# daxiongpro/EPNet

Hardware: AMD Instinct MI355X
Metric: SA-stack points/sec per GPU (16384-pt KITTI scene) + % HBM roofline (higher is better)
Workload: dtype f32; 1 GPU; 256 x 16384-pt kitti scenes per GPU per step through the 4-level SA op stack (4 samplings [FPS + centre gather; levels 2-4 nested in level 1 where tie-free] + 8 ball_query + 8 fused groupings [xyz - centre ; features]), pyramid 16384>4096>1024>256>64, radii [[.1,.5],[.5,1],[1,2],[2,4]], nsample [16,32], C=0/96/256/512, HIP-graph launch; levels=4, scenes_per_gpu=256, software_pipelined=True, pipeline_stages=2, parallelism=scene-parallel x1

## Files before the change

### epnet_amd/_lib.py

```python
import contextlib
import ctypes
import os

_HERE = os.path.dirname(os.path.abspath(__file__))
LIB_PATH = os.environ.get("EPNET_HIP_LIB") or os.path.join(_HERE, "lib", "libepnet_hip.so")

_vp = ctypes.c_void_p
_i = ctypes.c_int
_f = ctypes.c_float
_d = ctypes.c_double
_sz = ctypes.c_size_t
_i64 = ctypes.c_int64

SIGNATURES = {
    "epnet_abi_version": (_i, []),
    "epnet_strerror": (ctypes.c_char_p, [_i]),
    "epnet_last_hip_error": (ctypes.c_char_p, []),
    "epnet_set_tuning": (_i, [ctypes.c_char_p, _i]),
    "epnet_get_tuning": (_i, [ctypes.c_char_p, ctypes.POINTER(_i)]),
    "epnet_furthest_point_sampling": (_i, [_i, _i, _i, _vp, _vp, _vp, _vp]),
    "epnet_gather_points": (_i, [_i, _i, _i, _i, _vp, _vp, _vp, _vp]),
    "epnet_gather_points_grad": (_i, [_i, _i, _i, _i, _vp, _vp, _vp, _vp]),
    "epnet_ball_query": (_i, [_i, _i, _i, _f, _i, _vp, _vp, _vp, _vp]),
    "epnet_ball_query_workspace_bytes": (_sz, [_i, _i, _i]),
# ... 31 lines not shown
    "epnet_group_linear_grad_w_det_workspace_bytes": (_sz, [_i, _i, _i, _i]),
    "epnet_group_linear_grad_w_det": (_i, [_i, _i, _i, _i, _i, _vp, _vp, _vp, _vp, _vp, _vp, _sz, _vp]),
    "epnet_pool_max": (_i, [ctypes.c_longlong, _i, _vp, _vp, _vp, _vp]),
    "epnet_pool_max_grad": (_i, [ctypes.c_longlong, _i, _vp, _vp, _vp, _vp]),
    "epnet_group_linear_h": (_i, [_i, _i, _i, _i, _i, _vp, _vp, _vp, _vp, _vp, _vp, _vp, _i, _vp]),
    "epnet_pool_max_h": (_i, [ctypes.c_longlong, _i, _vp, _vp, _vp, _i, _vp]),
    "epnet_pool_max_grad_h": (_i, [ctypes.c_longlong, _i, _vp, _vp, _vp, _i, _vp]),
    "epnet_three_interpolate_h": (_i, [_i, _i, _i, _i, _vp, _vp, _vp, _vp, _i, _vp]),
    "epnet_scene_index_bytes": (_sz, [_i, _i]),
    "epnet_scene_index_build": (_i, [_i, _i, _vp, _vp, _sz, _vp]),
    "epnet_scene_index_build_gathered": (_i, [_i, _i, _i, _vp, _vp, _vp, _vp, _sz, _vp]),
    "epnet_furthest_point_sampling_indexed": (_i, [_i, _i, _i, _vp, _vp, _sz, _vp, _vp, _vp]),
    "epnet_sample_centres": (_i, [_i, _i, _i, _vp, _vp, _sz, _vp, _vp, _vp, _vp]),
    "epnet_sample_centres_chain": (_i, [_i, _i, _i, _vp, _vp, _sz, _vp, _vp, _vp, _vp, _vp, _i, _vp]),
    "epnet_sample_centres_chain_index": (_i, [_i, _i, _i, _vp, _vp, _sz, _vp, _vp, _vp, _vp, _vp, _i, _vp, _sz, _vp]),
    "epnet_group_concat_multi": (_i, [_i, _i, _i, _i, _i, _vp, _vp, _vp, _vp, _vp, _vp, _i, _vp]),
    "epnet_ball_query_indexed_multi": (_i, [_i, _i, _i, _i, _vp, _vp, _vp, _vp, _vp, _sz, _vp, _vp]),
    "epnet_ball_query_ordered": (_i, [_i, _i, _i, _i, _vp, _vp, _vp, _vp, _vp, _sz, _vp, _sz, _vp, _vp]),
    "epnet_three_nn_indexed": (_i, [_i, _i, _i, _vp, _vp, _vp, _sz, _vp, _sz, _vp, _vp, _vp]),
    "epnet_ball_query_indexed": (_i, [_i, _i, _i, _f, _i, _vp, _vp, _vp, _sz, _vp, _vp]),
    "epnet_boxes_overlap_bev": (_i, [_i, _vp, _i, _vp, _vp, _vp]),
    "epnet_boxes_iou_bev": (_i, [_i, _vp, _i, _vp, _vp, _vp]),
    "epnet_boxes_iou3d": (_i, [_i, _vp, _i, _vp, _vp, _vp]),
    "epnet_boxes_iou3d_pairs": (_i, [_i, _vp, _vp, _vp, _vp]),
    "epnet_aug_roi_by_noise": (_i, [_i, _i, _f, _vp, _vp, _vp, _vp, _vp, _vp, _vp, _vp]),
    "epnet_rcnn_sample_rois_workspace_bytes": (_sz, [_i, _i, _i, _i]),
    "epnet_rcnn_sample_rois": (_i, [_i, _i, _i, _i, _i, _i, _f, _f, _f, _d, _i, _vp, _vp, _vp, _vp, _vp, _vp, _vp, _sz, _vp, _vp, _vp,
                                    _vp, _vp, _vp, _vp, _vp, _vp, _vp]),
    "epnet_rpn_proposals_workspace_bytes": (_sz, [_i, _i, _i, _i]),
    "epnet_rpn_proposals": (_i, [_i, _i, _vp, _vp, _vp, _i, _i, _i, _f, _i, _vp, _sz, _vp, _vp, _vp, _vp]),
# ... 95 lines not shown
```

### epnet_amd/csrc/fps.hip

```cpp
#include <math.h>

#include <type_traits>

#include "common.h"
#include "dpp.h"
#include "spatial.h"

extern "C" __device__ int epnet_llvm_writelane_i32(int, int, int) __asm("llvm.amdgcn.writelane.i32");

namespace epnet {

__device__ __forceinline__ int writelane_i32(int value, int lane, int old) {
    return epnet_llvm_writelane_i32(value, lane, old);
}

__device__ __forceinline__ unsigned bitrev_lg(unsigned v, int lg) {
    return lg == 0 ? 0u : (__brev(v) >> (32 - lg));
}

__device__ __forceinline__ int wave_max_i32(int v) {
    const int r = row16_max(v);
    const int a = __builtin_amdgcn_readlane(r, 0), b = __builtin_amdgcn_readlane(r, 16);
    const int c = __builtin_amdgcn_readlane(r, 32), d = __builtin_amdgcn_readlane(r, 48);
    return max(max(a, b), max(c, d));
// ... 271 lines not shown
    if (PPT <= 8) a |= a >> 8;
    return (unsigned)a & (PPT >= 32 ? 0xFFFFFFFFu : ((1u << PPT) - 1u));
}

constexpr int kIdxBufP = 1024;

template <typename VH>
__device__ __forceinline__ unsigned rank_of(const VH &rk2, int j) {
    return ((unsigned)rk2[j >> 1] >> ((j & 1) << 4)) & 0xFFFFu;
}
template <typename VH>
__device__ __forceinline__ void set_rank(VH &rk2, int j, unsigned r) {
    rk2[j >> 1] = (j & 1) ? (int)(((unsigned)rk2[j >> 1] & 0xFFFFu) | (r << 16)) : (int)r;
}

template <int kW, int PPT, typename VF, typename VI, typename VH>
__device__ __forceinline__ void fps_rounds(unsigned long long *s_key, float4 (*s_rec)[64 * kW], int *s_idx, int m, const VF &x,
                                           const VF &y, const VF &z, VI &t, const VH &rk2,
                                           float cx, float cy, float cz, int *__restrict__ idxs,
                                           int *__restrict__ tie_free = nullptr, int known = 0,
                                           const float *__restrict__ xyz_in_order = nullptr, int detect_upto = 0x7fffffff) {
    const int q = threadIdx.x;
    const int lane = q & 63, wave = q >> 6;
    const int sub = lane & (PPT - 1);
    const int kNeg1 = __float_as_int(-1.f);

    int bm = kNeg1;
    float lox = 0.f, hix = 0.f, loy = 0.f, hiy = 0.f, loz = 0.f, hiz = 0.f;
    for (int j = 0; j < PPT; ++j) {
        const float xj = x[j], yj = y[j], zj = z[j];
        const int tj = t[j];
        const bool real = tj != kNeg1;
        const float mnx = group_minf<PPT>(real ? xj : 3.4e38f), mxx = group_maxf<PPT>(real ? xj : -3.4e38f);
        const float mny = group_minf<PPT>(real ? yj : 3.4e38f), mxy = group_maxf<PPT>(real ? yj : -3.4e38f);
        const float mnz = group_minf<PPT>(real ? zj : 3.4e38f), mxz = group_maxf<PPT>(real ? zj : -3.4e38f);
        const int gm = group_max<PPT>(tj);
        if (sub == j) {
            const bool any = gm != kNeg1;
            bm = gm;
            lox = any ? mnx : 0.f; hix = any ? mxx : 0.f;
            loy = any ? mny : 0.f; hiy = any ? mxy : 0.f;
            loz = any ? mnz : 0.f; hiz = any ? mxz : 0.f;
        }
    }
    if (q < 3) s_key[q] = 0ull;
    if (q == 0) s_idx[0] = 0;
    if (known > kIdxBufP || known > m || !xyz_in_order) known = 0;
    for (int i = q; i < known; i += 64 * kW) s_idx[i] = (int)rank14(i);
    __syncthreads();
    for (int it = 1; it < known; ++it) {
        const float px = __builtin_amdgcn_fmed3f(cx, lox, hix), py = __builtin_amdgcn_fmed3f(cy, loy, hiy),
                    pz = __builtin_amdgcn_fmed3f(cz, loz, hiz);
        const float bdx = px - cx, bdy = py - cy, bdz = pz - cz;
        const float L = bdx * bdx + bdy * bdy + bdz * bdz;
        unsigned active = fold_parts<PPT>(__ballot(__float_as_int(L) < bm));
        const float nx = xyz_in_order[it * 3 + 0], ny = xyz_in_order[it * 3 + 1], nz = xyz_in_order[it * 3 + 2];
        while (active) {
            const int j = (int)__builtin_ctz(active);
            active &= active - 1u;
            const float xj = x[j], yj = y[j], zj = z[j];
            const int told = t[j];
            __builtin_amdgcn_sched_barrier(0);
// ... 8 lines not shown
        cy = ny;
        cz = nz;
    }

    __builtin_amdgcn_s_setprio(EPNET_FPS_PRIO);
    EPNET_STATS_BEGIN;
    EPNET_STAMP(t_loop0);
    bool stale = true;
    int wbest = kNeg1;
    unsigned long long hbuckets = 0ull;
    unsigned racc = 0xFFFFFFFFu;
    float xa = 0.f, ya = 0.f, za = 0.f;
    int kb = 1;
    bool wave_multi = false;
    int tied_v = 0x7fffffff;
    auto round = [&](auto ties_tag, const int it) __attribute__((always_inline)) {
        constexpr bool kTies = decltype(ties_tag)::value;
        EPNET_STAMP(t0);
        const float px = __builtin_amdgcn_fmed3f(cx, lox, hix), py = __builtin_amdgcn_fmed3f(cy, loy, hiy),
                    pz = __builtin_amdgcn_fmed3f(cz, loz, hiz);
        const float bdx = px - cx, bdy = py - cy, bdz = pz - cz;
        const float L = bdx * bdx + bdy * bdy + bdz * bdz;
        const unsigned long long act64 = __ballot(__float_as_int(L) < bm);
        unsigned active = fold_parts<PPT>(act64);
        EPNET_CNT(0, __popc(active));
        stale = stale || __ballot((hbuckets & act64) != 0ull) != 0ull;
        EPNET_STAMP(t1);
        while (active) {
            const int j = (int)__builtin_ctz(active);
            active &= active - 1u;
            const float xj = x[j], yj = y[j], zj = z[j];
            const int told = t[j];
            __builtin_amdgcn_sched_barrier(0);
            const float dx = xj - cx, dy = yj - cy, dz = zj - cz;
            const float d = dx * dx + dy * dy + dz * dz;
            const int tj = min(__float_as_int(d), told);
            t[j] = tj;
            const int gm = group_max<PPT>(tj);
            bm = (sub == j) ? gm : bm;
        }
        EPNET_STAMP(t2);
        if (stale) {
            stale = false;
            wbest = wave_max_all(bm);
            unsigned cand = fold_parts<PPT>(__ballot(bm == wbest));
            racc = 0xFFFFFFFFu;
            hbuckets = 0ull;
            do {
                const int j = (int)__builtin_ctz(cand);
                cand &= cand - 1u;
                const int tj = t[j];
                const float xj = x[j], yj = y[j], zj = z[j];
                const unsigned rw = (unsigned)rk2[j >> 1];
                __builtin_amdgcn_sched_barrier(0);
                const unsigned r = tj == wbest ? ((rw >> ((j & 1) << 4)) & 0xFFFFu) : 0xFFFFFFFFu;
                if (r != 0xFFFFFFFFu) hbuckets |= 1ull << ((lane & ~(PPT - 1)) | j);
// ... 33 lines not shown
            const int wd = (int)(unsigned)(kfull >> 32);
            const bool suspect = (wbest == wd && (!mine || wave_multi)) || wd == 0;
            if (__builtin_amdgcn_readfirstlane(suspect ? 1 : 0)) {
                bool differs = false;
                const unsigned mine_slots = (unsigned)((hbuckets >> (lane & ~(PPT - 1))) & ((1ull << PPT) - 1ull));
                unsigned any_slots = mine_slots;
                for (int off = 32; off >= 1; off >>= 1) any_slots |= (unsigned)__shfl_xor((int)any_slots, off, 64);
#pragma unroll 1
                while (any_slots) {
                    const int j = (int)__builtin_ctz(any_slots);
                    any_slots &= any_slots - 1u;
                    const float xj = x[j], yj = y[j], zj = z[j];
                    __builtin_amdgcn_sched_barrier(0);
                    differs = differs || (((mine_slots >> j) & 1u) && (xj != cx || yj != cy || zj != cz));
                }
                if (wd == 0 || __ballot(differs)) tied_v = min(tied_v, it);
            }
        }
        const int kb2 = kb == 0 ? 2 : kb - 1;
        kb = kb == 2 ? 0 : kb + 1;
        if (wave == 0) {
            s_idx[it & (kIdxBufP - 1)] = (int)(0x3FFFu - (klo >> 10));
            if (lane == 0) s_key[kb2] = 0ull;
            if ((it & (kIdxBufP - 1)) == kIdxBufP - 1) {
                const int base = it - (kIdxBufP - 1);
                for (int e = lane; e < kIdxBufP; e += 64) idxs[base + e] = unrank14((unsigned)s_idx[e]);
            }
        }
        EPNET_STAMP(t5);
        EPNET_ACC(1, t0, t1); EPNET_ACC(2, t1, t2); EPNET_ACC(3, t2, t3); EPNET_ACC(4, t3, t4); EPNET_ACC(5, t4, t5);
    };
    int it0 = max(1, known);
    if (tie_free) {
        const int upto = min(m, detect_upto);
        for (; it0 < upto; ++it0) round(std::true_type{}, it0);
    }
    for (; it0 < m; ++it0) round(std::false_type{}, it0);
    EPNET_STAMP(t_loop1);
    EPNET_ACC(6, t_loop0, t_loop1);
    EPNET_STATS_END;
    if (tie_free && lane == 0) atomicMin(tie_free, min(min(tied_v, m), detect_upto));
    if (wave == 0) {
        const int base = (m - 1) & ~(kIdxBufP - 1);
        for (int e = lane; base + e < m; e += 64) idxs[base + e] = unrank14((unsigned)s_idx[e]);
    }
}

template <int kW, int PPT>
__global__ __launch_bounds__(64 * kW) void fps_pruned_kernel(int n, int m, const float *__restrict__ xyz,
                                                             float *__restrict__ temp, int *__restrict__ idxs,
                                                             const int *__restrict__ skip, int *__restrict__ prefix_out,
                                                             int prefix_cap) {
// ... 58 lines not shown

template <int kT, int BITS, int kPer, int kStage>
__device__ __attribute__((noinline)) void fps_index_epilogue(int *s_hist, float (*s_box)[16], int *s_part, int m, int np,
                                                             const float *xyz, float4 *sorted, float *boxes, float *qboxes, int n_src,
                                                             const int *src_idx, float *gathered) {
    scene_index_build_block<kT, BITS, kPer, kStage, true>(s_hist, s_box, s_part, m, np, xyz, sorted, boxes, qboxes, n_src, src_idx,
                                                          gathered);
}

template <int kW, int PPT>
__global__ __launch_bounds__(64 * kW) void fps_indexed_kernel(int n, int m, const float4 *__restrict__ sorted,
                                                              float *__restrict__ temp, int *__restrict__ idxs,
                                                              const int *__restrict__ prefix_in,
                                                              int *__restrict__ prefix_out, const float *__restrict__ xyz,
                                                              int prefix_cap, int prologue_init, void *next_index,
                                                              float *__restrict__ new_xyz) {
    typedef float vecf __attribute__((ext_vector_type(PPT)));
    typedef int veci __attribute__((ext_vector_type(PPT)));
    constexpr int NP = 64 * kW * PPT;
    constexpr bool kEpilogue = kW == 8;
    constexpr int kRecAt = 0, kIdxAt = kRecAt + 2 * 64 * kW * 16, kKeyAt = kIdxAt + kIdxBufP * 4, kFirstAt = kKeyAt + 32,
                  kRoundsBytes = kFirstAt + 16;
    constexpr int kIxBits = 12, kIxPer = 8, kIxStage = 512;
    constexpr int kIxHistWords = (1 << kIxBits) + (1 << kIxBits) / ((1 << kIxBits) / (64 * kW)) + 64;
    constexpr int kStageAt = kIxHistWords * 4, kBoxAt = kStageAt + kIxStage * 16, kPartAt = kBoxAt + 6 * 16 * 4,
                  kIxBytes = kEpilogue ? kPartAt + 16 * 4 : 0;
    constexpr int kArgsAt = kRoundsBytes;
    static_assert(kStageAt % 16 == 0 && kIxBytes <= 32768, "the sampling workgroup shares its CU with two 64 KB row gathers");
    static_assert(!kEpilogue || kArgsAt + 32 <= kIxBytes, "epilogue arguments");
    __shared__ __attribute__((aligned(16))) unsigned char s_lds[kRoundsBytes > kIxBytes ? kRoundsBytes : kIxBytes];
    unsigned long long *const s_key = reinterpret_cast<unsigned long long *>(s_lds + kKeyAt);
    float4(*const s_rec)[64 * kW] = reinterpret_cast<float4(*)[64 * kW]>(s_lds + kRecAt);
    int *const s_idx = reinterpret_cast<int *>(s_lds + kIdxAt);
    float *const s_first = reinterpret_cast<float *>(s_lds + kFirstAt);
    unsigned long long *const s_args = reinterpret_cast<unsigned long long *>(s_lds + kArgsAt);
    const int q = threadIdx.x;
    const int lane = q & 63, wave = q >> 6;
    const int known = prefix_in ? prefix_in[blockIdx.x] : 0;
    if (fps_prologue(m, prefix_in, idxs + (size_t)blockIdx.x * m, prefix_out, prologue_init)) return;
    sorted += (size_t)blockIdx.x * NP;
    if (temp) temp += (size_t)blockIdx.x * n;
    idxs += (size_t)blockIdx.x * m;
    typedef int vech __attribute__((ext_vector_type(PPT / 2)));
    vecf x, y, z;
    veci t;
    vech rk2;
#pragma unroll
    for (int j = 0; j < PPT; ++j) {
        const float4 v = sorted[((j * kW + wave) << 6) | lane];
        const int k = __float_as_int(v.w);
        if (k >= 0) {
            x[j] = v.x;
            y[j] = v.y;
            z[j] = v.z;
// ... 6 lines not shown
            }
        } else {
            x[j] = y[j] = z[j] = 0.f;
            t[j] = __float_as_int(-1.f);
            set_rank(rk2, j, 0xFFFFu);
        }
    }
    if constexpr (kEpilogue) {
        if (q == 0) {
            s_args[0] = (unsigned long long)next_index;
            s_args[1] = (unsigned long long)new_xyz;
            s_args[2] = (unsigned long long)xyz;
            s_args[3] = (unsigned long long)(unsigned)n;
        }
    }
    __syncthreads();
    fps_rounds<kW, PPT>(s_key, s_rec, s_idx, m, x, y, z, t, rk2, s_first[0], s_first[1], s_first[2], idxs,
                        prefix_out ? prefix_out + blockIdx.x : nullptr, known, xyz ? xyz + (size_t)blockIdx.x * n * 3 : nullptr,
                        prefix_cap);
    if (temp) {
#pragma unroll
        for (int j = 0; j < PPT; ++j) {
            const unsigned r = rank_of(rk2, j);
            if (r != 0xFFFFu) temp[unrank14(r)] = __int_as_float(t[j]);
        }
    }
    if constexpr (kEpilogue) {
        void *const next_index_ = (void *)s_args[0];
        if (next_index_) {
            float *const new_xyz_ = (float *)s_args[1];
            const float *const xyz_ = (const float *)s_args[2];
            const int n_ = (int)s_args[3];
            __threadfence_block();
            __syncthreads();
// ... 418 lines not shown
    float4 *dst = reinterpret_cast<float4 *>(out + ((size_t)bs * m + (size_t)i4 * 4) * 3);
    dst[0] = make_float4(a0, a1, a2, b0);
    dst[1] = make_float4(b1, b2, c0, c1);
    dst[2] = make_float4(c2, d0, d1, d2);
}

static void launch_gather_centres(int b, int n, int m, const float *xyz, const int *idx, float *new_xyz, hipStream_t s) {
    if ((m & 3) == 0 && (((uintptr_t)idx | (uintptr_t)new_xyz) & 15) == 0)
        hipLaunchKernelGGL(gather_centres4_kernel, dim3(div_up(m / 4, 256), b), dim3(256), 0, s, n, m, xyz, idx, new_xyz);
    else
        hipLaunchKernelGGL(gather_centres_kernel, dim3(div_up(m * 3, 256), b), dim3(256), 0, s, n, m, xyz, idx, new_xyz);
}

static int fps_over_index(int b, int n, int m, const float *xyz, void *index, size_t index_bytes, float *temp, int *idx,
                          float *new_xyz, hipStream_t s, const int *skip = nullptr, int *prefix_out = nullptr,
                          int prefix_cap = 0x7fffffff, void *next_index = nullptr, size_t next_index_bytes = 0) {
    const size_t need = scene_index_bytes(b, n);
    int rc;
    if (next_index) {
        const size_t need2 = scene_index_bytes(b, m);
        EPNET_REQUIRE(need2 != 0 && m <= 16384 && new_xyz && xyz && idx && b <= 65535);
        if (next_index_bytes < need2) return EPNET_ENOMEM;
        if (((uintptr_t)next_index & 15) != 0) return EPNET_EINVAL;
    }
    bool built_next = false;
    const bool plain = need == 0 || !index || n <= 1024 || m <= 1 || (n > 16384 && !temp);
    int fold_init = -1;
    bool wrote_centres = false;
    if (skip || prefix_out) {
        EPNET_REQUIRE(idx && b <= 65535);
        if (prefix_cap < 1) prefix_cap = 0x7fffffff;
        fold_init = fps_detects_ties(n, m, !plain) ? m : 0;
    }
// ... 12 lines not shown
            EPNET_REQUIRE(xyz);
            if (fold_init >= 0) {
                hipLaunchKernelGGL(fps_prefix_kernel, dim3(b), dim3(256), 0, s, m, skip, idx, prefix_out, fold_init);
                rc = check_launch("sampling prefix");
                if (rc) return rc;
            }
            const int np = scene_index_np(n);
            const float *bucket_boxes = (const float *)(sorted + (size_t)b * np);
            float *tsort = scene_index_sampling_scratch(b, n, index);
            hipLaunchKernelGGL(pruned::fps_bigscene_kernel<16>, grid, dim3(1024), 0, s, n, np, m, xyz, sorted, bucket_boxes, temp, tsort, idx, skip);
        } else {
            const bool epilogue = next_index && !skip && scene_index_np(n) == 16384 && m >= 1024 && m <= 4096;
            void *const epi_index = epilogue ? next_index : nullptr;
#define EPNET_FPS_INDEXED(W_, P_)                                                                                                     \
    hipLaunchKernelGGL((pruned::fps_indexed_kernel<W_, P_>), grid, dim3(64 * W_), 0, s, n, m, sorted, temp, idx, skip, prefix_out, xyz, \
                       prefix_cap, fold_init, epi_index, new_xyz)
            built_next = epilogue;
            switch (scene_index_np(n)) {
                case 2048: EPNET_FPS_INDEXED(4, 8); break;
                case 4096: EPNET_FPS_INDEXED(4, 16); break;
                case 8192: EPNET_FPS_INDEXED(4, 32); break;
                default: EPNET_FPS_INDEXED(8, 32); break;
            }
#undef EPNET_FPS_INDEXED
        }
        rc = check_launch("furthest_point_sampling");
    }
    if (rc || built_next) return rc;
    if (next_index) {
        const int np2 = scene_index_np(m);
        float4 *sorted2 = (float4 *)next_index;
// ... 31 lines not shown
    return fps_over_index(b, n, m, xyz, index, index_bytes, temp, idx, new_xyz, (hipStream_t)stream, prefix_in, prefix_out,
                          prefix_cap);
}

extern "C" int epnet_sample_centres_chain_index(int b, int n, int m, const float *xyz, void *index, size_t index_bytes,
                                                float *temp, int *idx, float *new_xyz, const int *prefix_in, int *prefix_out,
                                                int prefix_cap, void *next_index, size_t next_index_bytes,
                                                epnet_stream_t stream) {
    EPNET_REQUIRE(b >= 0 && n >= 1 && m >= 0);
    if (b == 0 || m == 0) return EPNET_OK;
    EPNET_REQUIRE(xyz && idx && new_xyz && next_index);
    if (m > n) prefix_in = nullptr;
    return fps_over_index(b, n, m, xyz, index, index_bytes, temp, idx, new_xyz, (hipStream_t)stream, prefix_in, prefix_out,
                          prefix_cap, next_index, next_index_bytes);
}
```

### epnet_amd/pointnet2_cuda.py

```python
import torch

from . import _lib
from ._tensor import ROWS16, dev_ptr, dev_ptr16, need, on_device_of, writes

_F, _I = torch.float32, torch.int32


def _deterministic():
    return torch.are_deterministic_algorithms_enabled()


def _det_call(l, name, ws_bytes, like, args, s, what):
    ws = torch.empty((max(int(ws_bytes), 1),), dtype=torch.uint8, device=like.device)
    _lib.check(getattr(l, "epnet_%s_det" % name)(*args, ws.data_ptr(), int(ws_bytes), s), "%s (deterministic)" % what)


@writes("idx")
def ball_query_wrapper(b, n, m, radius, nsample, new_xyz, xyz, idx):
    pn, px, pi = dev_ptr(new_xyz, "new_xyz", _F), dev_ptr(xyz, "xyz", _F), dev_ptr(idx, "idx", _I)
    need(new_xyz, b * m * 3, "new_xyz"); need(xyz, b * n * 3, "xyz"); need(idx, b * m * nsample, "idx")
    l = _lib.lib()
    ws_bytes = l.epnet_ball_query_workspace_bytes(b, n, m)
    with on_device_of(xyz) as s:
        if ws_bytes:
# ... 215 lines not shown
    px, nb = _index_args(index, points)
    nx, nnb = _index_args(next_index, points)
    if nx is None:
        raise RuntimeError("sample_centres_index_wrapper needs the next level's index buffer")
    pin = dev_ptr(prefix_in, "prefix_in", _I) if prefix_in is not None else None
    pout = dev_ptr(prefix_out, "prefix_out", _I) if prefix_out is not None else None
    if prefix_in is not None:
        need(prefix_in, b, "prefix_in")
    if prefix_out is not None:
        need(prefix_out, b, "prefix_out")
    temp = None if 64 <= n <= 16384 else torch.full((b, n), 1e10, dtype=_F, device=points.device)
    pt = None if temp is None else temp.data_ptr()
    with on_device_of(points) as s:
        _lib.check(_lib.lib().epnet_sample_centres_chain_index(b, n, m, pp, px, nb, pt, pi, pn, pin, pout, int(prefix_cap), nx, nnb, s),
                   "sample_centres_index")
    return 1


@writes("idxs")
def ball_query_multi_wrapper(b, n, m, radii, nsamples, new_xyz, xyz, index, idxs):
    import ctypes
    pn, pxyz = dev_ptr(new_xyz, "new_xyz", _F), dev_ptr(xyz, "xyz", _F)
    need(new_xyz, b * m * 3, "new_xyz"); need(xyz, b * n * 3, "xyz")
    k = len(radii)
    assert len(nsamples) == k and len(idxs) == k
    ptrs = []
    for ns, t in zip(nsamples, idxs):
        ptrs.append(dev_ptr(t, "idx", _I))
        need(t, b * m * ns, "idx")
    px, nb = _index_args(index, xyz)
# ... 261 lines not shown
```

### epnet_amd/sa_stack.py

```python
import os

import torch

from . import pointnet2_cuda as ext

RPN_NPOINTS = (4096, 1024, 256, 64)
RPN_RADII = ((0.1, 0.5), (0.5, 1.0), (1.0, 2.0), (2.0, 4.0))
RPN_NSAMPLES = ((16, 32), (16, 32), (16, 32), (16, 32))
RPN_FEAT_CHANNELS = (0, 96, 256, 512)
RPN_FP = ((1024, 64, 256), (512, 256, 1024), (512, 1024, 4096), (256, 4096, 16384))


CONFIGS = {
    2: dict(n=16384, npoints=RPN_NPOINTS, radii=RPN_RADII, nsamples=RPN_NSAMPLES, feat_channels=RPN_FEAT_CHANNELS),
    5: dict(n=65536, npoints=(16384,), radii=((0.5,),), nsamples=((64,),), feat_channels=(64,)),
}


def sa_algorithmic_bytes(n=16384, npoints=RPN_NPOINTS, nsamples=RPN_NSAMPLES, feat_channels=RPN_FEAT_CHANNELS):
    out = {"fps": 0, "gather": 0, "ball_query": 0, "group_xyz": 0, "group_feat": 0}
    cur = n
    for lvl, m in enumerate(npoints):
        out["fps"] += cur * 12 + m * 4
        out["gather"] += m * 4 + 3 * cur * 4 + 3 * m * 4
# ... 8 lines not shown
    return out


def fp_algorithmic_bytes(fp=RPN_FP):
    out = {"three_nn": 0, "three_interpolate": 0}
    for c, m, n in fp:
        out["three_nn"] += n * 12 + m * 12 + n * 24
        out["three_interpolate"] += c * m * 4 + n * 24 + c * n * 4
    out["total"] = sum(out.values())
    return out


class SAStack:
    def __init__(self, batch, n=16384, device="cuda", npoints=RPN_NPOINTS, radii=RPN_RADII, nsamples=RPN_NSAMPLES,
                 feat_channels=RPN_FEAT_CHANNELS, with_fp=False, fp=RPN_FP, seed=0, overlap=True, fused=True,
                 shared_index=True, pipelined=False, fused_sampling=False, queries_in_s=None, s_query_levels=None, stages=None):
        self.batch, self.n = batch, n
        if stages is None:
            stages = int(os.environ.get("EPNET_SA_STAGES", "2"))
        self.stages = 3 if (pipelined and stages == 3 and fused_sampling and fused and shared_index) else (2 if pipelined else 1)
        self.ring = self.stages
        self.overlap = overlap
        self.fused = fused
        self.shared_index = shared_index
        self.pipelined = pipelined
        self.fused_sampling = fused_sampling
        env_q = int(os.environ.get("EPNET_SA_QUERIES_IN_S", "1"))
        env_lv = os.environ.get("EPNET_SA_S_QUERY_LEVELS")
        every = frozenset(range(len(npoints)))
        if not pipelined:
            chosen = frozenset()
# ... 1 lines not shown
            chosen = frozenset(int(v) for v in s_query_levels)
        elif queries_in_s is not None:
            chosen = every if queries_in_s else frozenset()
        elif env_lv is not None:
            chosen = frozenset(int(v) for v in env_lv.split(",") if v.strip())
        elif self.stages == 3:
            chosen = every
        elif env_q == 2 or (env_q == 1 and with_fp):
            chosen = every
        elif env_q == 1 and batch * n >= 240 * 16384:
            chosen = every - {0, 1}
        else:
            chosen = frozenset()
        self.s_query_levels = chosen & every
        self.queries_in_s = self.s_query_levels == every
        self.chain = bool(int(os.environ.get("EPNET_SA_CHAIN", "1"))) and fused_sampling
        self.fuse_gather = int(os.environ.get("EPNET_SA_FUSE_GATHER", "1"))
        self._deferred = None
        self._next_built = None
        self.s_first = bool(int(os.environ.get("EPNET_SA_S_FIRST", "0" if self.s_query_levels else "1")))
        self.tail_scales = int(os.environ.get("EPNET_SA_TAIL_SCALES", "0"))
        self.multi_query = bool(int(os.environ.get("EPNET_SA_MULTI_QUERY", "1")))
        self.multi_group = bool(int(os.environ.get("EPNET_SA_MULTI_GROUP", "1")))
        self.ordered_query = bool(int(os.environ.get("EPNET_SA_ORDERED_QUERY", "1")))
        self.side = None
        self.npoints, self.radii, self.nsamples, self.feat_channels = npoints, radii, nsamples, feat_channels
        self.with_fp, self.fp = with_fp, fp
        dev = torch.device(device)
        g = torch.Generator().manual_seed(seed)
        f32, i32 = torch.float32, torch.int32
        self.levels = []
        cur = n
        for lvl, m in enumerate(npoints):
            c = feat_channels[lvl]
            index_bytes = ext.scene_index_bytes(batch, cur) if shared_index else 0
            L = {
                "n": cur, "m": m, "c": c,
                "xyz_t_sets": [torch.empty((batch, 3, cur), dtype=f32, device=dev) for _ in range(self.ring if not fused else 1)],
                "temp": torch.empty((batch, cur), dtype=f32, device=dev),
                "fps_idx_sets": ([torch.empty((batch, m), dtype=i32, device=dev) for _ in range(3)] if self.stages == 3 else None),
                "fps_idx": None,
                "new_xyz_t": torch.empty((batch, 3, m), dtype=f32, device=dev),
                "sets": [{"new_xyz": torch.empty((batch, m, 3), dtype=f32, device=dev),
                          "index": (torch.empty((index_bytes,), dtype=torch.uint8, device=dev) if index_bytes else None),
                          "prefix": torch.zeros((batch,), dtype=i32, device=dev),
                          "centre_index": (torch.empty((ext.scene_index_bytes(batch, m),), dtype=torch.uint8, device=dev)
                                           if (shared_index and lvl + 1 == len(npoints) and ext.scene_index_bytes(batch, m)) else None)}
                         for _ in range(self.ring)],
                "features": (torch.randn((batch, c, cur), generator=g, dtype=f32).to(dev) if c else None),
                "scales": [],
            }
            for radius, ns in zip(radii[lvl], nsamples[lvl]):
                S = {"radius": radius, "ns": ns, "idx": torch.empty((batch, m, ns), dtype=i32, device=dev)}
                S["idx_sets"] = [S["idx"]] + ([torch.empty((batch, m, ns), dtype=i32, device=dev) for _ in range(self.ring - 1)]
                                              if lvl in self.s_query_levels else [])
                if fused:
                    S["grouped"] = torch.empty((batch, 3 + c, m, ns), dtype=f32, device=dev)
                    ws_bytes = ext.group_concat_workspace_bytes(batch, c, cur, m, ns)
                    S["workspace"] = torch.empty((ws_bytes,), dtype=torch.uint8, device=dev) if ws_bytes else None
                else:
                    S["grouped_xyz"] = torch.empty((batch, 3, m, ns), dtype=f32, device=dev)
                    S["grouped_feat"] = torch.empty((batch, c, m, ns), dtype=f32, device=dev) if c else None
                L["scales"].append(S)
            if L["fps_idx_sets"] is None:
                one = torch.empty((batch, m), dtype=i32, device=dev)
                L["fps_idx_sets"] = [one] * self.ring
            L["fps_idx"] = L["fps_idx_sets"][0]
            self.levels.append(L)
            cur = m
        self.fp_bufs = []
        if with_fp:
            for c, m, nn_ in fp:
                sets = [{"dist2": torch.empty((batch, nn_, 3), dtype=f32, device=dev),
                         "idx": torch.empty((batch, nn_, 3), dtype=i32, device=dev),
                         "weight": torch.empty((batch, nn_, 3), dtype=f32, device=dev)} for _ in range(self.ring)]
                self.fp_bufs.append({
                    "c": c, "m": m, "n": nn_,
                    "known_feats": torch.randn((batch, c, m), generator=g, dtype=f32).to(dev),
                    "sets": sets,
                    "dist2": sets[0]["dist2"], "idx": sets[0]["idx"],
                    "out": torch.empty((batch, c, nn_), dtype=f32, device=dev),
                })
        self.graphs = []
        self.replays = 0
# ... 42 lines not shown
            prev = self.levels[lvl - 1]
            ext.scene_index_build_gathered_wrapper(b, prev["n"], n, src_xyz, prev["fps_idx_sets"][parity], cur_xyz, P["index"])
        elif built == (lvl, parity):
            pass
        elif P["index"] is not None and not index_built:
            ext.scene_index_build_wrapper(b, n, cur_xyz, P["index"])
        if self.fused_sampling:
            if not self.fused:
                L["xyz_t_sets"][parity].copy_(cur_xyz.transpose(1, 2))
            if self.chain:
                prefix_in = self.levels[lvl - 1]["sets"][parity]["prefix"] if lvl > 0 else None
                nxt = self.levels[lvl + 1]["m"] if lvl + 1 < len(self.levels) else 1
                nxt_L = self.levels[lvl + 1] if lvl + 1 < len(self.levels) else None
                defer = (defer_ok and self.fuse_gather and self.fused and nxt_L is not None
                         and nxt_L["sets"][parity]["index"] is not None and 1024 <= m <= 16384)
                if defer and self.fuse_gather == 1:
                    ext.sample_centres_index_wrapper(b, n, m, cur_xyz, P["index"], L["fps_idx_sets"][parity], P["new_xyz"],
                                                     nxt_L["sets"][parity]["index"], prefix_in, P["prefix"], nxt)
                    self._next_built = (lvl + 1, parity)
                else:
                    ext.sample_centres_wrapper(b, n, m, cur_xyz, P["index"], L["fps_idx_sets"][parity], None if defer else P["new_xyz"],
                                               prefix_in, P["prefix"], nxt)
                    if defer:
                        self._deferred = (cur_xyz, lvl, parity)
            else:
                ext.sample_centres_wrapper(b, n, m, cur_xyz, P["index"], L["fps_idx_sets"][parity], P["new_xyz"])
        else:
            L["xyz_t_sets"][parity if not self.fused else 0].copy_(cur_xyz.transpose(1, 2))
            L["temp"].fill_(1e10)
            if P["index"] is not None:
                ext.furthest_point_sampling_indexed_wrapper(b, n, m, cur_xyz, P["index"], L["temp"], L["fps_idx_sets"][parity])
# ... 96 lines not shown
        main = torch.cuda.current_stream(xyz.device)
        side = self._side_stream(xyz.device)
        first = self.levels[0]
        if first["sets"][parity]["index"] is not None:
            ext.scene_index_build_wrapper(self.batch, first["n"], xyz, first["sets"][parity]["index"])
        forked = torch.cuda.Event()
        forked.record(main)
        s_cur = xyz
        if self.s_first:
            s_cur = self._sample_level(first, xyz, parity, index_built=True, defer_ok=True)
        side.wait_event(forked)
        with torch.cuda.stream(side):
            inputs = [prev_xyz] + [L["sets"][1 - parity]["new_xyz"] for L in self.levels[:-1]]
            in_s = self.s_query_levels
            deep = list(enumerate(zip(self.levels, inputs)))[1:]
            for lvl, (L, cur) in deep[:1]:
                if lvl not in in_s:
                    self._query_level(L, cur, 1 - parity)
                self._group_scales(L, cur, 1 - parity)
            for lvl, (L, cur) in deep[1:]:
                if lvl not in in_s:
                    self._query_level(L, cur, 1 - parity)
            for lvl, (L, cur) in deep[1:]:
                self._group_scales(L, cur, 1 - parity)
            if 0 in in_s:
                self._group_scales(first, prev_xyz, 1 - parity)
            elif self.tail_scales == 0:
                self._group_level(first, prev_xyz, 1 - parity)
            else:
                for S in first["scales"][self.tail_scales:]:
                    self._query_scale(first, S, prev_xyz, 1 - parity)
                    self._group_scale(first, S, prev_xyz, 1 - parity)
            if self.with_fp:
                self._interpolate_fp(1 - parity)
        for L in self.levels[(1 if self.s_first else 0):]:
            s_cur = self._sample_level(L, s_cur, parity, index_built=L is first, defer_ok=True)
        if self.with_fp:
            self._search_fp(xyz, parity)
        if self.s_query_levels:
            self._queries_of(xyz, parity)
        for S in first["scales"][:(0 if 0 in self.s_query_levels else self.tail_scales)]:
            self._query_scale(first, S, prev_xyz, 1 - parity)
            self._group_scale(first, S, prev_xyz, 1 - parity)
        main.wait_stream(side)

    def run_pipelined3(self, clouds, step):
        p, q, r = step % 3, (step - 1) % 3, (step - 2) % 3
        main = torch.cuda.current_stream(clouds[p].device)
        side = self._side_stream(clouds[p].device)
        third = self._third_stream(clouds[p].device)
        first = self.levels[0]
        ext.scene_index_build_wrapper(self.batch, first["n"], clouds[p], first["sets"][p]["index"])
        forked = torch.cuda.Event()
        forked.record(main)
        self._deferred = self._next_built = None
        self._sample_level(first, clouds[p], p, index_built=True, defer_ok=True)
        s1_deferred = self._deferred is not None
        s1_built = self._next_built is not None
# ... 142 lines not shown
```

### include/epnet_ops.h

```cpp
#ifndef EPNET_OPS_H
#define EPNET_OPS_H

#include <stddef.h>
#include <stdint.h>

#ifdef __cplusplus
extern "C" {
#endif

#define EPNET_ABI_VERSION 1

#define EPNET_OK 0
#define EPNET_EINVAL (-1)
#define EPNET_ELAUNCH (-2)
#define EPNET_ENOMEM (-3)
#define EPNET_ELIMIT (-4)

typedef void *epnet_stream_t;

int epnet_abi_version(void);
const char *epnet_strerror(int code);
const char *epnet_last_hip_error(void);

int epnet_set_tuning(const char *name, int value);
// ... 108 lines not shown

size_t epnet_scene_index_bytes(int b, int n);
int epnet_scene_index_build(int b, int n, const float *xyz, void *index, size_t index_bytes, epnet_stream_t stream);
int epnet_scene_index_build_gathered(int b, int n_src, int n, const float *xyz_src, const int *idx, float *gathered, void *index,
                                     size_t index_bytes, epnet_stream_t stream);
int epnet_furthest_point_sampling_indexed(int b, int n, int m, const float *xyz, void *index,
                                          size_t index_bytes, float *temp, int *idx, epnet_stream_t stream);
int epnet_sample_centres(int b, int n, int m, const float *xyz, void *index, size_t index_bytes, float *temp,
                         int *idx, float *new_xyz, epnet_stream_t stream);
int epnet_sample_centres_chain(int b, int n, int m, const float *xyz, void *index, size_t index_bytes, float *temp,
                               int *idx, float *new_xyz, const int *prefix_in, int *prefix_out, int prefix_cap,
                               epnet_stream_t stream);
int epnet_sample_centres_chain_index(int b, int n, int m, const float *xyz, void *index, size_t index_bytes, float *temp,
                                     int *idx, float *new_xyz, const int *prefix_in, int *prefix_out, int prefix_cap,
                                     void *next_index, size_t next_index_bytes, epnet_stream_t stream);
int epnet_three_nn_indexed(int b, int n, int m, const float *unknown, const float *known, const void *unknown_index,
                           size_t unknown_index_bytes, const void *known_index, size_t known_index_bytes, float *dist2,
                           int *idx, epnet_stream_t stream);
int epnet_ball_query_indexed(int b, int n, int m, float radius, int nsample, const float *new_xyz, const float *xyz,
                             const void *index, size_t index_bytes, int *idx, epnet_stream_t stream);
int epnet_ball_query_indexed_multi(int b, int n, int m, int nscales, const float *radii, const int *nsamples,
                                   const float *new_xyz, const float *xyz, const void *index, size_t index_bytes,
                                   int *const *idx, epnet_stream_t stream);
int epnet_ball_query_ordered(int b, int n, int m, int nscales, const float *radii, const int *nsamples, const float *new_xyz,
                             const float *xyz, const void *index, size_t index_bytes, const void *centre_index,
                             size_t centre_index_bytes, int *const *idx, epnet_stream_t stream);


int epnet_boxes_overlap_bev(int num_a, const float *boxes_a, int num_b, const float *boxes_b,
                            float *ans_overlap, epnet_stream_t stream);
// ... 196 lines not shown
```

Measured before the change: 1.477 billion points/s.

## Log level-1 FPS ties and skip selection rounds in level-2 nested sampling

```diff
diff --git a/epnet_amd/_lib.py b/epnet_amd/_lib.py
--- a/epnet_amd/_lib.py
+++ b/epnet_amd/_lib.py
@@ -69,6 +69,7 @@
     "epnet_sample_centres": (_i, [_i, _i, _i, _vp, _vp, _sz, _vp, _vp, _vp, _vp]),
     "epnet_sample_centres_chain": (_i, [_i, _i, _i, _vp, _vp, _sz, _vp, _vp, _vp, _vp, _vp, _i, _vp]),
     "epnet_sample_centres_chain_index": (_i, [_i, _i, _i, _vp, _vp, _sz, _vp, _vp, _vp, _vp, _vp, _i, _vp, _sz, _vp]),
+    "epnet_sample_centres_chain_ties": (_i, [_i, _i, _i, _vp, _vp, _sz, _vp, _vp, _vp, _vp, _vp, _i, _vp, _vp, _vp, _vp, _sz, _vp]),
     "epnet_group_concat_multi": (_i, [_i, _i, _i, _i, _i, _vp, _vp, _vp, _vp, _vp, _vp, _i, _vp]),
     "epnet_ball_query_indexed_multi": (_i, [_i, _i, _i, _i, _vp, _vp, _vp, _vp, _vp, _sz, _vp, _vp]),
     "epnet_ball_query_ordered": (_i, [_i, _i, _i, _i, _vp, _vp, _vp, _vp, _vp, _sz, _vp, _sz, _vp, _vp]),
diff --git a/epnet_amd/csrc/fps.hip b/epnet_amd/csrc/fps.hip
--- a/epnet_amd/csrc/fps.hip
+++ b/epnet_amd/csrc/fps.hip
@@ -309,12 +309,20 @@
     rk2[j >> 1] = (j & 1) ? (int)(((unsigned)rk2[j >> 1] & 0xFFFFu) | (r << 16)) : (int)r;
 }
 
-template <int kW, int PPT, typename VF, typename VI, typename VH>
+constexpr int kTieRounds = 1024, kTieWords = kTieRounds / 32;
+__device__ __forceinline__ unsigned tie_words_unwatched(int watched, int w) {
+    const int lo = w * 32;
+    return watched <= lo ? 0xFFFFFFFFu : (watched >= lo + 32 ? 0u : 0xFFFFFFFFu << (watched - lo));
+}
+
+template <int kW, int PPT, bool kInterleave = false, typename VF, typename VI, typename VH>
 __device__ __forceinline__ void fps_rounds(unsigned long long *s_key, float4 (*s_rec)[64 * kW], int *s_idx, int m, const VF &x,
                                            const VF &y, const VF &z, VI &t, const VH &rk2,
                                            float cx, float cy, float cz, int *__restrict__ idxs,
                                            int *__restrict__ tie_free = nullptr, int known = 0,
-                                           const float *__restrict__ xyz_in_order = nullptr, int detect_upto = 0x7fffffff) {
+                                           const float *__restrict__ xyz_in_order = nullptr, int detect_upto = 0x7fffffff,
+                                           unsigned *s_ties = nullptr, const unsigned *__restrict__ ties_in = nullptr,
+                                           float *s_pre = nullptr, int *__restrict__ real_rounds_out = nullptr) {
     const int q = threadIdx.x;
     const int lane = q & 63, wave = q >> 6;
     const int sub = lane & (PPT - 1);
@@ -341,6 +349,18 @@
     if (q < 3) s_key[q] = 0ull;
     if (q == 0) s_idx[0] = 0;
     if (known > kIdxBufP || known > m || !xyz_in_order) known = 0;
+    if (s_ties && (unsigned)(q - 64) < (unsigned)kTieWords) s_ties[q - 64] = 0u;
+    bool follow = false;
+    unsigned tin = 0u;
+    if constexpr (kInterleave) {
+        follow = ties_in && xyz_in_order && m <= kTieRounds;
+        if (follow) tin = ties_in[lane & (kTieWords - 1)];
+        if (follow) {
+            for (int i = q; i < m; i += 64 * kW) s_idx[i] = (int)rank14(i);
+            for (int e = q; e < m * 3; e += 64 * kW) s_pre[e] = xyz_in_order[e];
+            known = 0;
+        }
+    }
     for (int i = q; i < known; i += 64 * kW) s_idx[i] = (int)rank14(i);
     __syncthreads();
     for (int it = 1; it < known; ++it) {
@@ -379,8 +399,11 @@
     int kb = 1;
     bool wave_multi = false;
     int tied_v = 0x7fffffff;
-    auto round = [&](auto ties_tag, const int it) __attribute__((always_inline)) {
-        constexpr bool kTies = decltype(ties_tag)::value;
+    int won_pick = 0;
+    bool won_positive = false;
+    unsigned long long st_t0 = 0ull, st_t1 = 0ull, st_t2 = 0ull;
+    (void)st_t0, (void)st_t1, (void)st_t2;
+    auto update = [&](const int it) __attribute__((always_inline)) {
         EPNET_STAMP(t0);
         const float px = __builtin_amdgcn_fmed3f(cx, lox, hix), py = __builtin_amdgcn_fmed3f(cy, loy, hiy),
                     pz = __builtin_amdgcn_fmed3f(cz, loz, hiz);
@@ -405,6 +428,15 @@
             bm = (sub == j) ? gm : bm;
         }
         EPNET_STAMP(t2);
+#ifdef EPNET_FPS_STATS
+        st_t0 = t0, st_t1 = t1, st_t2 = t2;
+#endif
+    };
+    auto select = [&](auto ties_tag, const int it) __attribute__((always_inline)) {
+        constexpr bool kTies = decltype(ties_tag)::value;
+#ifdef EPNET_FPS_STATS
+        const unsigned long long t0 = st_t0, t1 = st_t1, t2 = st_t2;
+#endif
         if (stale) {
             stale = false;
             wbest = wave_max_all(bm);
@@ -468,8 +500,16 @@
                     __builtin_amdgcn_sched_barrier(0);
                     differs = differs || (((mine_slots >> j) & 1u) && (xj != cx || yj != cy || zj != cz));
                 }
-                if (wd == 0 || __ballot(differs)) tied_v = min(tied_v, it);
-            }
+                const bool tie = wd == 0 || __ballot(differs);
+                if (tie) tied_v = min(tied_v, it);
+                if (s_ties)
+                    __hip_atomic_fetch_or(&s_ties[(it >> 5) & (kTieWords - 1)], tie && it < kTieRounds ? 1u << (it & 31) : 0u,
+                                          __ATOMIC_RELAXED, __HIP_MEMORY_SCOPE_WORKGROUP);
+            }
+        }
+        if constexpr (kInterleave) {
+            won_pick = unrank14(0x3FFFu - (klo >> 10));
+            won_positive = (int)(unsigned)(kfull >> 32) > 0;
         }
         const int kb2 = kb == 0 ? 2 : kb - 1;
         kb = kb == 2 ? 0 : kb + 1;
@@ -485,11 +525,49 @@
         EPNET_ACC(1, t0, t1); EPNET_ACC(2, t1, t2); EPNET_ACC(3, t2, t3); EPNET_ACC(4, t3, t4); EPNET_ACC(5, t4, t5);
     };
     int it0 = max(1, known);
-    if (tie_free) {
-        const int upto = min(m, detect_upto);
-        for (; it0 < upto; ++it0) round(std::true_type{}, it0);
-    }
-    for (; it0 < m; ++it0) round(std::false_type{}, it0);
+    int real_rounds = m - it0;
+    auto round = [&](auto ties_tag, const int it) __attribute__((always_inline)) {
+        update(it);
+        select(ties_tag, it);
+    };
+    if (kInterleave && follow) {
+        const int upto = tie_free ? min(m, detect_upto) : 0;
+        bool closed = true;
+        int seg_max = 0;
+        real_rounds = 0;
+        for (; it0 < m; ++it0) {
+            const bool marked = ((unsigned)__builtin_amdgcn_readlane((int)tin, (it0 >> 5) & (kTieWords - 1)) >> (it0 & 31)) & 1u;
+            const bool selecting = !closed || marked;
+            const float nx = s_pre[it0 * 3 + 0], ny = s_pre[it0 * 3 + 1], nz = s_pre[it0 * 3 + 2];
+            if (selecting && closed) {
+                __syncthreads();
+                if (q < 3) s_key[q] = 0ull;
+                stale = true;
+                closed = false;
+                seg_max = 0;
+                __syncthreads();
+            }
+            update(it0);
+            if (!selecting) {
+                cx = nx;
+                cy = ny;
+                cz = nz;
+                continue;
+            }
+            if (it0 < upto) select(std::true_type{}, it0);
+            else select(std::false_type{}, it0);
+            ++real_rounds;
+            seg_max = max(seg_max, won_pick);
+            closed = won_positive && seg_max <= it0;
+        }
+    } else {
+        if (tie_free) {
+            const int upto = min(m, detect_upto);
+            for (; it0 < upto; ++it0) round(std::true_type{}, it0);
+        }
+        for (; it0 < m; ++it0) round(std::false_type{}, it0);
+    }
+    if (real_rounds_out && q == 0) *real_rounds_out = real_rounds;
     EPNET_STAMP(t_loop1);
     EPNET_ACC(6, t_loop0, t_loop1);
     EPNET_STATS_END;
@@ -578,7 +656,8 @@
                                                               const int *__restrict__ prefix_in,
                                                               int *__restrict__ prefix_out, const float *__restrict__ xyz,
                                                               int prefix_cap, int prologue_init, void *next_index,
-                                                              float *__restrict__ new_xyz) {
+                                                              float *__restrict__ new_xyz, const unsigned *__restrict__ ties_in,
+                                                              unsigned *__restrict__ ties_out, int *__restrict__ real_rounds_out) {
     typedef float vecf __attribute__((ext_vector_type(PPT)));
     typedef int veci __attribute__((ext_vector_type(PPT)));
     constexpr int NP = 64 * kW * PPT;
@@ -589,10 +668,13 @@
     constexpr int kIxHistWords = (1 << kIxBits) + (1 << kIxBits) / ((1 << kIxBits) / (64 * kW)) + 64;
     constexpr int kStageAt = kIxHistWords * 4, kBoxAt = kStageAt + kIxStage * 16, kPartAt = kBoxAt + 6 * 16 * 4,
                   kIxBytes = kEpilogue ? kPartAt + 16 * 4 : 0;
-    constexpr int kArgsAt = kRoundsBytes;
-    static_assert(kStageAt % 16 == 0 && kIxBytes <= 32768, "the sampling workgroup shares its CU with two 64 KB row gathers");
-    static_assert(!kEpilogue || kArgsAt + 32 <= kIxBytes, "epilogue arguments");
-    __shared__ __attribute__((aligned(16))) unsigned char s_lds[kRoundsBytes > kIxBytes ? kRoundsBytes : kIxBytes];
+    constexpr bool kInterleave = kW == 4 && PPT <= 16;
+    constexpr int kArgsAt = kRoundsBytes, kTiesAt = kArgsAt + 48, kPreAt = kTiesAt + kTieWords * 4,
+                  kAllBytes = kPreAt + (kInterleave ? kTieRounds * 12 : 0);
+    static_assert(kStageAt % 16 == 0 && kIxBytes <= 32768 && kAllBytes <= 32768, "the sampling workgroup shares its CU with two 64 KB row gathers");
+    __shared__ __attribute__((aligned(16))) unsigned char s_lds[kAllBytes > kIxBytes ? kAllBytes : kIxBytes];
+    unsigned *const s_ties = reinterpret_cast<unsigned *>(s_lds + kTiesAt);
+    float *const s_pre = kInterleave ? reinterpret_cast<float *>(s_lds + kPreAt) : nullptr;
     unsigned long long *const s_key = reinterpret_cast<unsigned long long *>(s_lds + kKeyAt);
     float4(*const s_rec)[64 * kW] = reinterpret_cast<float4(*)[64 * kW]>(s_lds + kRecAt);
     int *const s_idx = reinterpret_cast<int *>(s_lds + kIdxAt);
@@ -601,7 +683,12 @@
     const int q = threadIdx.x;
     const int lane = q & 63, wave = q >> 6;
     const int known = prefix_in ? prefix_in[blockIdx.x] : 0;
-    if (fps_prologue(m, prefix_in, idxs + (size_t)blockIdx.x * m, prefix_out, prologue_init)) return;
+    if (fps_prologue(m, prefix_in, idxs + (size_t)blockIdx.x * m, prefix_out, prologue_init)) {
+        if (ties_out && q < kTieWords)
+            ties_out[(size_t)blockIdx.x * kTieWords + q] = tie_words_unwatched(prefix_out ? min(m, prefix_cap) : 0, q);
+        if (real_rounds_out && q == 0) real_rounds_out[blockIdx.x] = 0;
+        return;
+    }
     sorted += (size_t)blockIdx.x * NP;
     if (temp) temp += (size_t)blockIdx.x * n;
     idxs += (size_t)blockIdx.x * m;
@@ -638,10 +725,23 @@
             s_args[3] = (unsigned long long)(unsigned)n;
         }
     }
+    if (q == 0) {
+        s_args[4] = (unsigned long long)(ties_out ? ties_out + (size_t)blockIdx.x * kTieWords : nullptr);
+        s_args[5] = (unsigned long long)(unsigned)(prefix_out ? min(m, prefix_cap) : 0);
+    }
     __syncthreads();
-    fps_rounds<kW, PPT>(s_key, s_rec, s_idx, m, x, y, z, t, rk2, s_first[0], s_first[1], s_first[2], idxs,
-                        prefix_out ? prefix_out + blockIdx.x : nullptr, known, xyz ? xyz + (size_t)blockIdx.x * n * 3 : nullptr,
-                        prefix_cap);
+    fps_rounds<kW, PPT, kInterleave>(s_key, s_rec, s_idx, m, x, y, z, t, rk2, s_first[0], s_first[1], s_first[2], idxs,
+                                     prefix_out ? prefix_out + blockIdx.x : nullptr, known,
+                                     xyz ? xyz + (size_t)blockIdx.x * n * 3 : nullptr, prefix_cap, s_ties,
+                                     kInterleave && ties_in ? ties_in + (size_t)blockIdx.x * kTieWords : nullptr, s_pre,
+                                     kInterleave && real_rounds_out ? real_rounds_out + blockIdx.x : nullptr);
+    {
+        unsigned *const ties_out_ = (unsigned *)s_args[4];
+        if (ties_out_) {
+            __syncthreads();
+            if (q < kTieWords) ties_out_[q] = s_ties[q] | tie_words_unwatched((int)s_args[5], q);
+        }
+    }
     if (temp) {
 #pragma unroll
         for (int j = 0; j < PPT; ++j) {
@@ -1090,9 +1190,14 @@
 
 static int fps_over_index(int b, int n, int m, const float *xyz, void *index, size_t index_bytes, float *temp, int *idx,
                           float *new_xyz, hipStream_t s, const int *skip = nullptr, int *prefix_out = nullptr,
-                          int prefix_cap = 0x7fffffff, void *next_index = nullptr, size_t next_index_bytes = 0) {
+                          int prefix_cap = 0x7fffffff, void *next_index = nullptr, size_t next_index_bytes = 0,
+                          const unsigned *ties_in = nullptr, unsigned *ties_out = nullptr, int *real_rounds_out = nullptr) {
     const size_t need = scene_index_bytes(b, n);
     int rc;
+    if (ties_in || ties_out || real_rounds_out) {
+        EPNET_REQUIRE(need != 0 && index && n > 1024 && n <= 16384 && m > 1 && b <= 65535);
+        EPNET_REQUIRE(!real_rounds_out || scene_index_np(n) <= 4096);
+    }
     if (next_index) {
         const size_t need2 = scene_index_bytes(b, m);
         EPNET_REQUIRE(need2 != 0 && m <= 16384 && new_xyz && xyz && idx && b <= 65535);
@@ -1135,7 +1240,7 @@
             void *const epi_index = epilogue ? next_index : nullptr;
 #define EPNET_FPS_INDEXED(W_, P_)                                                                                                     \
     hipLaunchKernelGGL((pruned::fps_indexed_kernel<W_, P_>), grid, dim3(64 * W_), 0, s, n, m, sorted, temp, idx, skip, prefix_out, xyz, \
-                       prefix_cap, fold_init, epi_index, new_xyz)
+                       prefix_cap, fold_init, epi_index, new_xyz, ties_in, ties_out, real_rounds_out)
             built_next = epilogue;
             switch (scene_index_np(n)) {
                 case 2048: EPNET_FPS_INDEXED(4, 8); break;
@@ -1197,3 +1302,15 @@
     return fps_over_index(b, n, m, xyz, index, index_bytes, temp, idx, new_xyz, (hipStream_t)stream, prefix_in, prefix_out,
                           prefix_cap, next_index, next_index_bytes);
 }
+
+extern "C" int epnet_sample_centres_chain_ties(int b, int n, int m, const float *xyz, void *index, size_t index_bytes, float *temp,
+                                               int *idx, float *new_xyz, const int *prefix_in, int *prefix_out, int prefix_cap,
+                                               const unsigned *ties_in, unsigned *ties_out, int *real_rounds_out, void *next_index,
+                                               size_t next_index_bytes, epnet_stream_t stream) {
+    EPNET_REQUIRE(b >= 0 && n >= 1 && m >= 0);
+    if (b == 0 || m == 0) return EPNET_OK;
+    EPNET_REQUIRE(xyz && idx && (new_xyz || !next_index));
+    if (m > n) prefix_in = nullptr, ties_in = nullptr;
+    return fps_over_index(b, n, m, xyz, index, index_bytes, temp, idx, new_xyz, (hipStream_t)stream, prefix_in, prefix_out,
+                          prefix_cap, next_index, next_index_bytes, ties_in, ties_out, real_rounds_out);
+}
diff --git a/epnet_amd/pointnet2_cuda.py b/epnet_amd/pointnet2_cuda.py
--- a/epnet_amd/pointnet2_cuda.py
+++ b/epnet_amd/pointnet2_cuda.py
@@ -253,6 +253,32 @@
     with on_device_of(points) as s:
         _lib.check(_lib.lib().epnet_sample_centres_chain_index(b, n, m, pp, px, nb, pt, pi, pn, pin, pout, int(prefix_cap), nx, nnb, s),
                    "sample_centres_index")
+    return 1
+
+
+TIE_WORDS = 32
+
+
+@writes("idx", "new_xyz", "prefix_out", "next_index", "ties_out", "real_rounds_out")
+def sample_centres_ties_wrapper(b, n, m, points, index, idx, new_xyz, next_index=None, prefix_in=None, prefix_out=None, prefix_cap=0,
+                                ties_in=None, ties_out=None, real_rounds_out=None):
+    pp, pi = dev_ptr(points, "points", _F), dev_ptr(idx, "idx", _I)
+    pn = dev_ptr(new_xyz, "new_xyz", _F) if new_xyz is not None else None
+    need(points, b * n * 3, "points"); need(idx, b * m, "idx")
+    if new_xyz is not None:
+        need(new_xyz, b * m * 3, "new_xyz")
+    px, nb = _index_args(index, points)
+    nx, nnb = _index_args(next_index, points)
+    ptrs = []
+    for t, name, count in ((prefix_in, "prefix_in", b), (prefix_out, "prefix_out", b), (ties_in, "ties_in", b * TIE_WORDS),
+                           (ties_out, "ties_out", b * TIE_WORDS), (real_rounds_out, "real_rounds_out", b)):
+        if t is not None:
+            need(t, count, name)
+        ptrs.append(dev_ptr(t, name, _I) if t is not None else None)
+    pin, pout, tin, tout, rr = ptrs
+    with on_device_of(points) as s:
+        _lib.check(_lib.lib().epnet_sample_centres_chain_ties(b, n, m, pp, px, nb, None, pi, pn, pin, pout, int(prefix_cap), tin, tout, rr,
+                                                              nx, nnb, s), "sample_centres_ties")
     return 1
 
 
diff --git a/epnet_amd/sa_stack.py b/epnet_amd/sa_stack.py
--- a/epnet_amd/sa_stack.py
+++ b/epnet_amd/sa_stack.py
@@ -46,7 +46,8 @@
 class SAStack:
     def __init__(self, batch, n=16384, device="cuda", npoints=RPN_NPOINTS, radii=RPN_RADII, nsamples=RPN_NSAMPLES,
                  feat_channels=RPN_FEAT_CHANNELS, with_fp=False, fp=RPN_FP, seed=0, overlap=True, fused=True,
-                 shared_index=True, pipelined=False, fused_sampling=False, queries_in_s=None, s_query_levels=None, stages=None):
+                 shared_index=True, pipelined=False, fused_sampling=False, queries_in_s=None, s_query_levels=None, stages=None,
+                 s_group_levels=None):
         self.batch, self.n = batch, n
         if stages is None:
             stages = int(os.environ.get("EPNET_SA_STAGES", "2"))
@@ -78,6 +79,9 @@
             chosen = frozenset()
         self.s_query_levels = chosen & every
         self.queries_in_s = self.s_query_levels == every
+        env_g = os.environ.get("EPNET_SA_S_GROUP_LEVELS", "")
+        picked = s_group_levels if s_group_levels is not None else [v for v in env_g.split(",") if v.strip()]
+        self.s_group_levels = (frozenset(int(v) for v in picked) & every) if (pipelined and self.stages == 2) else frozenset()
         self.chain = bool(int(os.environ.get("EPNET_SA_CHAIN", "1"))) and fused_sampling
         self.fuse_gather = int(os.environ.get("EPNET_SA_FUSE_GATHER", "1"))
         self._deferred = None
@@ -108,6 +112,7 @@
                 "sets": [{"new_xyz": torch.empty((batch, m, 3), dtype=f32, device=dev),
                           "index": (torch.empty((index_bytes,), dtype=torch.uint8, device=dev) if index_bytes else None),
                           "prefix": torch.zeros((batch,), dtype=i32, device=dev),
+                          "ties": (torch.zeros((batch, ext.TIE_WORDS), dtype=i32, device=dev) if lvl == 0 else None),
                           "centre_index": (torch.empty((ext.scene_index_bytes(batch, m),), dtype=torch.uint8, device=dev)
                                            if (shared_index and lvl + 1 == len(npoints) and ext.scene_index_bytes(batch, m)) else None)}
                          for _ in range(self.ring)],
@@ -132,6 +137,9 @@
             L["fps_idx"] = L["fps_idx_sets"][0]
             self.levels.append(L)
             cur = m
+        self.tie_log = (bool(int(os.environ.get("EPNET_SA_TIE_LOG", "1"))) and self.chain and len(self.levels) > 1
+                        and 1024 < n <= 16384 and 1024 < npoints[0] <= 4096 and 1 < npoints[1] <= 1024
+                        and self.levels[0]["sets"][0]["index"] is not None and self.levels[1]["sets"][0]["index"] is not None)
         self.fp_bufs = []
         if with_fp:
             for c, m, nn_ in fp:
@@ -204,7 +212,18 @@
                 nxt_L = self.levels[lvl + 1] if lvl + 1 < len(self.levels) else None
                 defer = (defer_ok and self.fuse_gather and self.fused and nxt_L is not None
                          and nxt_L["sets"][parity]["index"] is not None and 1024 <= m <= 16384)
-                if defer and self.fuse_gather == 1:
+                ties_out = P["ties"] if (self.tie_log and lvl == 0) else None
+                ties_in = self.levels[0]["sets"][parity]["ties"] if (self.tie_log and lvl == 1) else None
+                if ties_in is not None or ties_out is not None:
+                    nx = nxt_L["sets"][parity]["index"] if (defer and self.fuse_gather == 1) else None
+                    ext.sample_centres_ties_wrapper(b, n, m, cur_xyz, P["index"], L["fps_idx_sets"][parity],
+                                                    None if (defer and nx is None) else P["new_xyz"], nx, prefix_in, P["prefix"], nxt,
+                                                    ties_in, ties_out)
+                    if nx is not None:
+                        self._next_built = (lvl + 1, parity)
+                    elif defer:
+                        self._deferred = (cur_xyz, lvl, parity)
+                elif defer and self.fuse_gather == 1:
                     ext.sample_centres_index_wrapper(b, n, m, cur_xyz, P["index"], L["fps_idx_sets"][parity], P["new_xyz"],
                                                      nxt_L["sets"][parity]["index"], prefix_in, P["prefix"], nxt)
                     self._next_built = (lvl + 1, parity)
@@ -331,16 +350,30 @@
             inputs = [prev_xyz] + [L["sets"][1 - parity]["new_xyz"] for L in self.levels[:-1]]
             in_s = self.s_query_levels
             deep = list(enumerate(zip(self.levels, inputs)))[1:]
+            in_s_tail = self.s_group_levels
+            queried = {}
+
+            def query(lvl, L, cur):
+                self._query_level(L, cur, 1 - parity)
+                if lvl in in_s_tail:
+                    queried[lvl] = torch.cuda.Event()
+                    queried[lvl].record(side)
+
             for lvl, (L, cur) in deep[:1]:
                 if lvl not in in_s:
-                    self._query_level(L, cur, 1 - parity)
-                self._group_scales(L, cur, 1 - parity)
+                    query(lvl, L, cur)
+                if lvl not in in_s_tail:
+                    self._group_scales(L, cur, 1 - parity)
             for lvl, (L, cur) in deep[1:]:
                 if lvl not in in_s:
-                    self._query_level(L, cur, 1 - parity)
+                    query(lvl, L, cur)
             for lvl, (L, cur) in deep[1:]:
-                self._group_scales(L, cur, 1 - parity)
-            if 0 in in_s:
+                if lvl not in in_s_tail:
+                    self._group_scales(L, cur, 1 - parity)
+            if 0 in in_s_tail and self.tail_scales == 0:
+                if 0 not in in_s:
+                    query(0, first, prev_xyz)
+            elif 0 in in_s:
                 self._group_scales(first, prev_xyz, 1 - parity)
             elif self.tail_scales == 0:
                 self._group_level(first, prev_xyz, 1 - parity)
@@ -359,6 +392,13 @@
         for S in first["scales"][:(0 if 0 in self.s_query_levels else self.tail_scales)]:
             self._query_scale(first, S, prev_xyz, 1 - parity)
             self._group_scale(first, S, prev_xyz, 1 - parity)
+        g_inputs = [prev_xyz] + [L["sets"][1 - parity]["new_xyz"] for L in self.levels[:-1]]
+        for lvl in sorted(self.s_group_levels):
+            if lvl == 0 and self.tail_scales != 0:
+                continue
+            if lvl in queried:
+                main.wait_event(queried[lvl])
+            self._group_scales(self.levels[lvl], g_inputs[lvl], 1 - parity)
         main.wait_stream(side)
 
     def run_pipelined3(self, clouds, step):
diff --git a/include/epnet_ops.h b/include/epnet_ops.h
--- a/include/epnet_ops.h
+++ b/include/epnet_ops.h
@@ -146,6 +146,10 @@
 int epnet_sample_centres_chain_index(int b, int n, int m, const float *xyz, void *index, size_t index_bytes, float *temp,
                                      int *idx, float *new_xyz, const int *prefix_in, int *prefix_out, int prefix_cap,
                                      void *next_index, size_t next_index_bytes, epnet_stream_t stream);
+int epnet_sample_centres_chain_ties(int b, int n, int m, const float *xyz, void *index, size_t index_bytes, float *temp,
+                                    int *idx, float *new_xyz, const int *prefix_in, int *prefix_out, int prefix_cap,
+                                    const unsigned *ties_in, unsigned *ties_out, int *real_rounds_out, void *next_index,
+                                    size_t next_index_bytes, epnet_stream_t stream);
 int epnet_three_nn_indexed(int b, int n, int m, const float *unknown, const float *known, const void *unknown_index,
                            size_t unknown_index_bytes, const void *known_index, size_t known_index_bytes, float *dist2,
                            int *idx, epnet_stream_t stream);
```

Result: no change. 1.486 billion points/s, median of 6 (+0.6%).
